# NGWPC/topoflow-glacier

Measured on AMD Instinct MI355X. Metric: cell-updates/sec (nx·ny·steps) on 8192² fp32 grid; % HBM roofline, higher is better.
Workload: dtype f32

## Files before the change

topoflow-glacier_amd/csrc/tfg_engine.hip:

```cpp
#include <hip/hip_runtime.h>
#include <mutex>

#include <algorithm>
#include <cmath>
#include <cstdio>
#include <cstdlib>
#include <atomic>
#include <chrono>
#include <cstring>
#include <new>
#include <string>
#include <type_traits>
#include <vector>

#include "../../include/tfg.h"
#include "tfg_physics.hpp"
#include "tfg_conduction.hpp"
#include "tfg_fused.hpp"
#include "tfg_hostbuf.hpp"

namespace {

using namespace tfg_kern;

// ... 978 lines not shown
  a.n_pad = h->n_pad;
  a.n_step = h->n_pad;
  return a;
}

template <class R, bool EXACT>
int launch_fused(tfg_handle* h, const tfg_uniforms* d_u, const StepAddr* d_t, int K, int blocks, size_t lds,
                 const IoArgs& io, bool ns, const Part* part = nullptr) {
  const hipStream_t stream = part ? part->stream : h->stream;
  KArgs a = step_args(h, K, io);
  if (part) {
    a.n = part->n_valid;
    a.n_step = part->cells;
  }
  const int64_t c0 = part ? part->c0 : 0;
  a.part_c0 = c0;
  const size_t rb = (size_t)c0 * h->rsz;
  const FusedBufs fb = {d_u, d_t, h->forc.bytes() + rb, h->stat.bytes() + rb, h->geo + c0,
                        h->catch_id ? h->catch_id + c0 : nullptr, h->st + c0, h->tot + c0, h->ring + c0,
                        h->hist.bytes() + rb, h->slab + (part ? part->slab_row0 : 0) * h->n_catch * 6,
                        h->qc ? h->qc.bytes() + rb : nullptr};
  const bool rd = !h->depths_derived;
  const bool ct = h->catch_id != nullptr;
  if constexpr (EXACT) {
    HIPCHK(h, launch_fused_exact(a, fb, rd, ct, h->qc_on, blocks, lds, stream));
    return TFG_OK;
  } else {
    const bool sat = h->dp.satterlund != 0;
    hipError_t e;
    if (h->flux_f64) e = sat ? launch_fused_fast<true, true>(a, fb, rd, ct, h->qc_on, ns, blocks, lds, stream)
                             : launch_fused_fast<true, false>(a, fb, rd, ct, h->qc_on, ns, blocks, lds, stream);
    else e = sat ? launch_fused_fast<false, true>(a, fb, rd, ct, h->qc_on, ns, blocks, lds, stream)
                 : launch_fused_fast<false, false>(a, fb, rd, ct, h->qc_on, ns, blocks, lds, stream);
    HIPCHK(h, e);
    return TFG_OK;
  }
}

}

template hipError_t tfg_kern::launch_fused_fast<false, false>(const KArgs&, const FusedBufs&, bool, bool, bool, bool, int,
                                                              size_t, hipStream_t);

extern "C" {

int tfg_abi_version(void) { return TFG_ABI_VERSION; }

#ifndef TFG_SRC_HASH
#define TFG_SRC_HASH "unknown"
#endif
#define TFG_STR2(x) #x
#define TFG_STR(x) TFG_STR2(x)
#if !defined(__HIP_DEVICE_COMPILE__)
__attribute__((used)) static const char tfg_build_tag[] =
    "libtfg abi=" TFG_STR(TFG_ABI_VERSION) " arch=gfx950 (hipcc) tfg-src-sha256=" TFG_SRC_HASH
    "; kernels: k_fused<float|double,exact|fast,...>, k_cell, k_cell_run, k_cell_many, k_diag_reduce, k_catch_series, k_band_series, k_forcing_expand, k_forcing_regrid, k_fill_synthetic";

const char* tfg_build_info(void) { return tfg_build_tag; }
#else
const char* tfg_build_info(void);
#endif

int tfg_device_count(int* count) {
  if (!count) return fail(nullptr, TFG_ERR_ARG, "null count");
  HIPCHK(nullptr, hipGetDeviceCount(count));
  return TFG_OK;
}

constexpr int64_t kPlaneSkew = 512;

int tfg_create(const tfg_params* p, int64_t ny, int64_t nx, int engine, int device, int n_frames,
               int hist_depth, int n_catch, tfg_handle** out) {
  if (!p || !out) return fail(nullptr, TFG_ERR_ARG, "null params/out");
  *out = nullptr;
  if (ny <= 0 || nx <= 0) return fail(nullptr, TFG_ERR_ARG, "grid must have ny, nx >= 1");
  if (ny > (1ll << 31) || nx > (1ll << 31))
    return fail(nullptr, TFG_ERR_ARG, "shard too large: ny and nx must stay below 2^31");
  if (engine != TFG_F32 && engine != TFG_F64) return fail(nullptr, TFG_ERR_ARG, "engine must be TFG_F32 or TFG_F64");
  if (n_frames < 1 || hist_depth < 1 || n_catch < 1) return fail(nullptr, TFG_ERR_ARG, "n_frames, hist_depth, n_catch must be >= 1");
  if (n_catch > 512) return fail(nullptr, TFG_ERR_ARG, "n_catch > 512 not supported");
  if (p->ring_len < 1) return fail(nullptr, TFG_ERR_ARG, "ring_len must be >= 1");
  if (!(p->dt > 0)) return fail(nullptr, TFG_ERR_ARG, "dt must be > 0");
  if (!(p->z0_air > 0.0 && p->z0_air < INFINITY)) return fail(nullptr, TFG_ERR_ARG, "z0_air must be finite and > 0");
  tfg_handle* h = new (std::nothrow) tfg_handle();
  if (!h) return fail(nullptr, TFG_ERR_ARG, "out of host memory");
  auto bail = [&](int rc) {
    g_err = h->err;
    tfg_destroy(h);
    return rc;
  };
  h->device = device;
  h->engine = engine;
  h->rsz = dtype_size(engine);
  h->ny = ny;
  h->nx = nx;
  h->n = ny * nx;
  h->n_pad = round_up(h->n, 64);
  h->n_pad += h->n_pad >= ((int64_t)1 << 20) ? kPlaneSkew : 0;
  if (h->n_pad * 8 >= (int64_t)1 << 32) {
    h->err = "shard too large: ny*nx must stay below 2^29 cells per device (32-bit field offsets)";
    g_err = h->err;
    delete h;
    return TFG_ERR_ARG;
  }
  h->n_frames = n_frames;
  h->hist_depth = hist_depth;
  h->n_catch = n_catch;
  h->ring_len = p->ring_len;
  derive_params(*p, h->dp);
  {
    const double rg = p->rho_ice * p->g;
    h->flow_gamma = 2.0 * p->glens_A / 5.0 * (rg * rg * rg);
    h->inv_cs = 1.0 / (p->rho_snow * p->Cp_snow);
    h->inv_ci = 1.0 / ((p->rho_ice * p->Cp_ice) * p->h_active_layer);
    h->h_active = p->h_active_layer;
  }
  if (hipSetDevice(device) != hipSuccess) { h->err = "hipSetDevice failed"; return bail(TFG_ERR_HIP); }
  hipDeviceProp_t prop;
  if (hipGetDeviceProperties(&prop, device) != hipSuccess) { h->err = "hipGetDeviceProperties failed"; return bail(TFG_ERR_HIP); }
  h->max_blocks = std::max(256, prop.multiProcessorCount * 512);
  h->max_blocks = (int)std::max<int64_t>(256, std::min<int64_t>(h->max_blocks, (256ll << 20) / ((int64_t)n_catch * 6 * 8)));
  while (h->max_blocks & (h->max_blocks - 1)) h->max_blocks &= h->max_blocks - 1;
  h->max_blocks = (int)std::min<int64_t>(h->max_blocks, (h->n_pad / kCellsPerThread + kBlock - 1) / kBlock);
  if (h->own_stream.create() != hipSuccess) { h->err = "stream create failed"; return bail(TFG_ERR_HIP); }
  h->stream = h->own_stream;
  const int64_t np = h->n_pad;
  const size_t rs = h->rsz;
  struct A { Buf<DevMem>* b; size_t bytes; } allocs[] = {
      {&h->forc, (size_t)n_frames * kNumForc * np * rs},
      {&h->stat, 3 * (size_t)np * rs},
      {&h->lwsw, 2 * (size_t)np * rs},
      {&h->geo, engine == TFG_F32 ? (size_t)np * (tfg::kGeoF * 4 + 2 * 8) : (size_t)np * tfg::kStaticPlanes * 8},
      {&h->st, (size_t)kNumState * np * 8},
      {&h->tot, (size_t)np * 8},
      {&h->ring, (size_t)p->ring_len * np * 4},
      {&h->hist, (size_t)hist_depth * kNumHist * np * rs},
      {&h->diag, (size_t)n_catch * 6 * 8},
      {&h->slab, (size_t)h->max_blocks * n_catch * 6 * 8},
      {&h->d_flag, (size_t)n_frames * kNumForc * 4},
  };
  for (auto& a : allocs) {
    const hipError_t e = (hipError_t)a.b->reserve(a.bytes);
    if (e != hipSuccess) {
      h->err = std::string("hipMalloc(") + std::to_string(a.bytes) + " B) failed: " + hipGetErrorString(e);
      return bail(TFG_ERR_HIP);
    }
    if (hipMemsetAsync(a.b->ptr, 0, a.bytes, h->stream) != hipSuccess) { h->err = "hipMemset failed"; return bail(TFG_ERR_HIP); }
  }
  if (hipStreamSynchronize(h->stream) != hipSuccess) { h->err = "sync failed"; return bail(TFG_ERR_HIP); }
  h->plane_state.assign((size_t)n_frames * kNumForc, kOk);
  *out = h;
  return TFG_OK;
}

int tfg_destroy(tfg_handle* h) {
  if (!h) return TFG_OK;
  (void)hipSetDevice(h->device);
  if (h->stream && h->stream != h->own_stream) (void)hipStreamSynchronize(h->stream);
  if (h->own_stream) (void)hipStreamSynchronize(h->own_stream);
  if (h->side) (void)hipStreamSynchronize(h->side);
  delete h;
  return TFG_OK;
}

int tfg_set_stream(tfg_handle* h, void* stream) {
  if (int rc_ = api_sync(h)) return rc_;
// ... 1563 lines not shown
```

topoflow-glacier_amd/csrc/tfg_fused.hpp:

```cpp
#pragma once

#include <hip/hip_runtime.h>

#include <algorithm>
#include <cmath>
#include <cstddef>
#include <cstdint>

#include "../../include/tfg.h"
#include "tfg_physics.hpp"

namespace tfg_kern {

using tfg::CellDiag;
using tfg::CellOut;
using tfg::CellState;
using tfg::CellStatic;
using tfg::CellStaticF;
using tfg::DevParams;

constexpr int kBlock = 256;
constexpr int kCellsPerThread = 1;
constexpr int kPrefetchFast = 2;
constexpr int kWaves = kBlock / 64;
// ... 89 lines not shown
#pragma unroll
    for (int off = 32; off >= 1; off >>= 1) {
      v0 += __shfl_xor(v0, off);
      v1 += __shfl_xor(v1, off);
      v2 += __shfl_xor(v2, off);
      v3 += __shfl_xor(v3, off);
      v4 += __shfl_xor(v4, off);
      m = tfg::npmax(m, __shfl_xor(m, off));
    }
    if (lane == leader) {
      double* b = wbins + 6 * c;
      b[0] += v0; b[1] += v1; b[2] += v2; b[3] += v3; b[4] += v4;
      b[5] = tfg::npmax(b[5], m);
    }
    pending &= ~__ballot(mine);
  }
}

#ifdef TFG_WG_TIMING
static __device__ unsigned long long g_wg_times[TFG_WG_TIMING][3];
#endif
constexpr int kMinWaves = 4;
constexpr int kMinWavesExact = 2;
constexpr int kMinWavesPrec = 4;
template <class R, bool EXACT, bool READ_DEPTHS, bool CATCH, bool QC, int C, bool NS = false, bool PREC = false,
          bool SAT = false>
__global__ __launch_bounds__(kBlock, EXACT ? kMinWavesExact : (PREC ? kMinWavesPrec : kMinWaves)) void k_fused(const KArgs a, const tfg_uniforms* __restrict__ uni,
                                                  const StepAddr* __restrict__ tab,
                                                  const R* __restrict__ forc,
                                                  const R* __restrict__ stat,
                                                  const float* __restrict__ geo,
                                                  const int32_t* __restrict__ catch_id,
                                                  double* __restrict__ st,
                                                  int64_t* __restrict__ tot,
                                                  int32_t* __restrict__ ring,
                                                  R* __restrict__ hist,
                                                  double* __restrict__ slab,
                                                  const R* __restrict__ qcf) {
  extern __shared__ double lds_bins[];
#ifdef TFG_WG_TIMING
  const unsigned long long t_wg0 = wall_clock64();
#endif
  const DevParams& p = a.p;
  const int nb = a.n_catch * 6;
  for (int i = threadIdx.x; i < kWaves * nb; i += kBlock) lds_bins[i] = ((i % 6) == 5) ? -INFINITY : 0.0;
  __syncthreads();
  double* wbins = lds_bins + (threadIdx.x >> 6) * nb;

  const int64_t n_pad = a.n_pad;
  const int64_t ngroups = a.n_step / C;
  const int64_t nchunks = (ngroups + kBlock - 1) / kBlock;
  const int64_t wg = blockIdx.x;
  const int64_t g0 = (wg * nchunks / gridDim.x) * kBlock;
  const int64_t g1 = std::min<int64_t>(((wg + 1) * nchunks / gridDim.x) * kBlock, ngroups);
  const int64_t trips = (g1 - g0 + kBlock - 1) / kBlock;
  const double* geo_d = reinterpret_cast<const double*>(geo + tfg::kGeoF * n_pad) + a.part_c0 / 2;
  float* const alb_f = reinterpret_cast<float*>(st + S_ALB * n_pad) - a.part_c0;

  CellDiag acc;
  diag_zero(acc);
  constexpr bool kAccLds = !EXACT && !CATCH;
  __shared__ double acc_lds[kAccLds ? 6 * kBlock : 1];
  auto acc_get = [&]() {
    const double* s = acc_lds + threadIdx.x;
    return CellDiag{s[0], s[kBlock], s[2 * kBlock], s[3 * kBlock], s[4 * kBlock], s[5 * kBlock]};
  };
  auto acc_put = [&](const CellDiag& d) {
    double* s = acc_lds + threadIdx.x;
    s[0] = d.P; s[kBlock] = d.PR; s[2 * kBlock] = d.PS; s[3 * kBlock] = d.SM; s[4 * kBlock] = d.IM; s[5 * kBlock] = d.Pmax;
  };
  if constexpr (kAccLds) acc_put(acc);

  for (int64_t it = 0; it < trips; ++it) {
    const int64_t g = g0 + it * kBlock + threadIdx.x;
    const bool in = g < g1;
    int32_t cid[C];
    CellDiag cacc[CATCH ? C : 1];
    if constexpr (CATCH) {
#pragma unroll
      for (int j = 0; j < C; ++j) { diag_zero(cacc[j]); cid[j] = 0; }
    }
    if (in) {
      const int64_t c0 = g * C;
      const uint32_t lc = (uint32_t)c0;
      CellStatic SX[EXACT ? C : 1];
      tfg::CellStaticF SF[EXACT ? 1 : C];
      if constexpr (EXACT) {
        const double* gx = reinterpret_cast<const double*>(geo);
        double v[tfg::kStaticPlanes][C];
#pragma unroll
        for (int f = 0; f < tfg::kStaticPlanes; ++f) dload<C>(gx + f * n_pad, lc, v[f]);
#pragma unroll
        for (int j = 0; j < C; ++j) SX[j] = {v[0][j], v[1][j], v[2][j], v[3][j], v[4][j], v[5][j], v[6][j]};
      } else {
        float gv[tfg::kGeoF][C];
#pragma unroll
        for (int f = 0; f < tfg::kGeoF; ++f) vload<float, C>(geo + f * n_pad, lc, gv[f]);
#pragma unroll
        for (int j = 0; j < C; ++j) SF[j] = {gv[0][j], gv[1][j], gv[2][j], gv[3][j], gv[4][j]};
      }
      CellState cs[C];
      {
        double v[C];
        dload<C>(st + S_HSWE * n_pad, lc, v);
#pragma unroll
        for (int j = 0; j < C; ++j) cs[j].h_swe = v[j];
        dload<C>(st + S_HIWE * n_pad, lc, v);
#pragma unroll
        for (int j = 0; j < C; ++j) cs[j].h_iwe = v[j];
        dload<C>(st + S_ECCS * n_pad, lc, v);
#pragma unroll
        for (int j = 0; j < C; ++j) cs[j].Eccs = v[j];
        dload<C>(st + S_ECCI * n_pad, lc, v);
#pragma unroll
        for (int j = 0; j < C; ++j) cs[j].Ecci = v[j];
        dload<C>(st + S_N * n_pad, lc, v);
#pragma unroll
        for (int j = 0; j < C; ++j) cs[j].n = v[j];
        if constexpr (EXACT) {
          dload<C>(st + S_ALB * n_pad, lc, v);
#pragma unroll
          for (int j = 0; j < C; ++j) cs[j].albedo = v[j];
        }
        if constexpr (READ_DEPTHS) {
          dload<C>(st + S_HSNOW * n_pad, lc, v);
#pragma unroll
          for (int j = 0; j < C; ++j) cs[j].h_snow = v[j];
          dload<C>(st + S_HICE * n_pad, lc, v);
#pragma unroll
          for (int j = 0; j < C; ++j) cs[j].h_ice = v[j];
        } else {
#pragma unroll
          for (int j = 0; j < C; ++j) {
            cs[j].h_snow = cs[j].h_swe * p.ws;
            cs[j].h_ice = cs[j].h_iwe * p.wi;
          }
        }
        int64_t t[C];
        lload<C>(tot, lc, t);
#pragma unroll
        for (int j = 0; j < C; ++j) cs[j].tot_q = t[j];
        if constexpr (!EXACT) {
          bool carried = false;
#pragma unroll
          for (int j = 0; j < C; ++j) {
            cs[j].albedo = 0.0;
            carried |= !(cs[j].h_snow > 0.0 || (cs[j].h_snow == 0.0 && (cs[j].h_ice > 0.0 || cs[j].h_ice == 0.0)));
          }
          if (__any(carried)) {
            float fa[C];
            vload<float, C>(alb_f, lc, fa);
#pragma unroll
            for (int j = 0; j < C; ++j) cs[j].albedo = (double)fa[j];
          }
        }
      }
      R qc[C];
      if constexpr (QC) vload<R, C>(qcf, lc, qc);
      else {
#pragma unroll
        for (int j = 0; j < C; ++j) qc[j] = (R)0;
      }
      tfg::DiagF df[EXACT ? 1 : C];
      if constexpr (!EXACT) {
#pragma unroll
        for (int j = 0; j < C; ++j) df[j] = {0.0f, 0.0f, 0.0f, 0.0f, 0.0f, 0.0f};
      }

      struct Frame { R P[C], T[C], Q[C], PA[C], UZ[C]; int32_t q[C]; };
      const char* const fbase = a.io_in ? static_cast<const char*>(a.io_in) : reinterpret_cast<const char*>(forc);
      auto fetch = [&](int k, Frame& f) {
        const StepAddr* ta = tab + (k < a.K ? k : a.K - 1);
        const int64_t fo = ta->forc, ro = ta->ring;
        const R* __restrict__ fr = reinterpret_cast<const R*>(fbase + fo);
        const int32_t* rs = reinterpret_cast<const int32_t*>(reinterpret_cast<const char*>(ring) + ro);
        static_assert(C == 1, "streamed step accesses are per cell");
        static_assert(sizeof(R) == 4 || sizeof(R) == 8, "R is float or double");
        const uint32_t oR = lane_off(lc * (uint32_t)sizeof(R));
        f.P[0] = sload(fr + F_P * n_pad, oR);
        f.T[0] = sload(fr + F_T * n_pad, oR);
        f.Q[0] = sload(fr + F_Q * n_pad, oR);
        f.PA[0] = sload(fr + F_PA * n_pad, oR);
        f.UZ[0] = sload(fr + F_UZ * n_pad, oR);
        f.q[0] = sload(rs, sizeof(R) == 4 ? oR : lane_off(lc * 4u));
      };
      auto advance = [&](int k, const Frame& f) {
        TFG_STEP_PARAMS(p);
        const tfg_uniforms* up = uni + k;
        const tfg_uniforms u = *up;
        int32_t qn[C];
        R o_hs[C], o_sm[C], o_hi[C], o_im[C], o_mt[C], o_rh[C];
#pragma unroll
        for (int j = 0; j < C; ++j) {
          if constexpr (EXACT) {
            CellOut o;
            CellDiag& d = CATCH ? cacc[j] : acc;
            const bool valid = (c0 + j) < a.n;
            const tfg::ParamsAsIs params{p};
            tfg::cell_step_exact<QC>(p, SX[j], u, (double)f.P[j], (double)f.T[j], (double)f.Q[j], (double)f.PA[j],
                                     (double)f.UZ[j], f.q[j], qn[j], cs[j], o, d, valid, (double)qc[j], params);
            o_hs[j] = (R)o.h_snow; o_sm[j] = (R)o.SM; o_hi[j] = (R)o.h_ice;
            o_im[j] = (R)o.IM; o_mt[j] = (R)o.M_total; o_rh[j] = (R)o.RH;
          } else {
            tfg::CellOutF o;
            tfg::cell_step_fast<QC, NS, PREC, SAT>(p, SF[j], up, u, geo_d, n_pad, c0 + j, (float)f.P[j], (float)f.T[j],
                                                   (float)f.Q[j], (float)f.PA[j], (float)f.UZ[j], f.q[j], qn[j], cs[j],
                                                   o, df[j], (float)qc[j]);
            o_hs[j] = (R)o.h_snow; o_sm[j] = (R)o.SM; o_hi[j] = (R)o.h_ice;
            o_im[j] = (R)o.IM; o_mt[j] = (R)o.M_total; o_rh[j] = (R)o.RH;
            asm volatile("" : "+v"(df[j].P), "+v"(df[j].PR), "+v"(df[j].PS), "+v"(df[j].Pmax));
          }
        }
        const uint32_t oR = lane_off(lc * (uint32_t)sizeof(R));
        const int64_t ro = tab[k].ring, ho = tab[k].hist;
        sstore(reinterpret_cast<int32_t*>(reinterpret_cast<char*>(ring) + ro), sizeof(R) == 4 ? oR : lane_off(lc * 4u), qn[0]);
        R* __restrict__ h = reinterpret_cast<R*>(reinterpret_cast<char*>(hist) + ho);
        sstore(h + H_HSNOW * n_pad, oR, o_hs[0]);
        sstore(h + H_SM * n_pad, oR, o_sm[0]);
        sstore(h + H_HICE * n_pad, oR, o_hi[0]);
        sstore(h + H_IM * n_pad, oR, o_im[0]);
        sstore(h + H_MTOT * n_pad, oR, o_mt[0]);
        sstore(h + H_RH * n_pad, oR, o_rh[0]);
      };
      constexpr int kAhead = (QC || NS || PREC) ? 1 : kPrefetchFast;
      Frame fa, fb;
      fetch(0, fa);
      if constexpr (EXACT) {
        for (int k = 0; k < a.K; ++k) {
          fetch(k + 1, fb);
          advance(k, fa);
          fa = fb;
        }
      } else if constexpr (kAhead == 2) {
        Frame fc;
        fetch(1, fb);
        int k = 0;
        if (a.K >= 3) {
          fetch(2, fc);
          advance(0, fa);
          fetch(3, fa);
          advance(1, fb);
          fetch(4, fb);
          advance(2, fc);
          for (k = 3; k + 3 <= a.K; k += 3) {
            fetch(k + 2, fc);
            advance(k, fa);
            fetch(k + 3, fa);
            advance(k + 1, fb);
            fetch(k + 4, fb);
            advance(k + 2, fc);
          }
        }
        if (k < a.K) {
          advance(k, fa);
          if (k + 1 < a.K) advance(k + 1, fb);
        }
      } else if constexpr (PREC && CATCH) {
        for (int k = 0; k < a.K; k += 2) {
          fetch(k + 1, fb);
          advance(k, fa);
          fetch(k + 2, fa);
          if (k + 1 < a.K) advance(k + 1, fb);
        }
      } else {
        int k = 0;
        if (a.K >= 2) {
          fetch(1, fb);
          advance(0, fa);
          fetch(2, fa);
          advance(1, fb);
          for (k = 2; k + 2 <= a.K; k += 2) {
            fetch(k + 1, fb);
            advance(k, fa);
            fetch(k + 2, fa);
            advance(k + 1, fb);
          }
        }
        if (k < a.K) advance(k, fa);
      }
      if (a.io_in) {
        const int fidx = uni[0].frame, hidx = uni[0].hist;
        R* __restrict__ fr = const_cast<R*>(forc) + (int64_t)fidx * kNumForc * n_pad;
        const uint32_t oR = lane_off(lc * (uint32_t)sizeof(R));
        sstore(fr + F_P * n_pad, oR, fa.P[0]);
        sstore(fr + F_T * n_pad, oR, fa.T[0]);
        sstore(fr + F_Q * n_pad, oR, fa.Q[0]);
        sstore(fr + F_PA * n_pad, oR, fa.PA[0]);
        sstore(fr + F_UZ * n_pad, oR, fa.UZ[0]);
        if (c0 < a.n) {
          const R* hs = hist + (int64_t)hidx * kNumHist * n_pad + c0;
          double* o = a.io_out + c0;
          const int64_t n = a.n;
          o[0 * n] = (double)hs[H_HSNOW * n_pad];
          o[1 * n] = cs[0].h_swe;
          o[2 * n] = (double)hs[H_SM * n_pad];
          o[3 * n] = (double)hs[H_HICE * n_pad];
          o[4 * n] = cs[0].h_iwe;
          o[5 * n] = (double)hs[H_IM * n_pad];
          o[6 * n] = (double)hs[H_MTOT * n_pad];
          o[7 * n] = (double)hs[H_RH * n_pad];
        }
      }
      if constexpr (CATCH) iload<C>(catch_id, lc, cid);
      if constexpr (!EXACT) {
        const double fP = p.da_m2 * p.dt, fSM = p.inv_dt_rhoLf * p.da_m2 * p.dt * 3600.0,
                     fIM = p.da_m2 * p.dt * 3600.0;
#pragma unroll
        for (int j = 0; j < C; ++j) {
          if ((c0 + j) < a.n) {
            CellDiag lsum;
            if constexpr (kAccLds) lsum = acc_get();
            CellDiag& d = CATCH ? cacc[j] : (kAccLds ? lsum : acc);
            d.P += (double)df[j].P * fP;
            d.PR += (double)df[j].PR * fP;
            d.PS += (double)df[j].PS * fP;
            d.SM += (double)df[j].Erem_s * fSM;
            d.IM += (double)df[j].IM * fIM;
            d.Pmax = tfg::npmax(d.Pmax, (double)df[j].Pmax);
            if constexpr (kAccLds) acc_put(lsum);
          }
        }
      }
      {
        double v[C];
#pragma unroll
        for (int j = 0; j < C; ++j) v[j] = cs[j].h_swe;
        dstore<C>(st + S_HSWE * n_pad, lc, v);
#pragma unroll
        for (int j = 0; j < C; ++j) v[j] = cs[j].h_iwe;
        dstore<C>(st + S_HIWE * n_pad, lc, v);
#pragma unroll
        for (int j = 0; j < C; ++j) v[j] = cs[j].Eccs;
        dstore<C>(st + S_ECCS * n_pad, lc, v);
#pragma unroll
        for (int j = 0; j < C; ++j) v[j] = cs[j].Ecci;
        dstore<C>(st + S_ECCI * n_pad, lc, v);
#pragma unroll
        for (int j = 0; j < C; ++j) v[j] = cs[j].n;
        dstore<C>(st + S_N * n_pad, lc, v);
        if constexpr (EXACT) {
#pragma unroll
          for (int j = 0; j < C; ++j) v[j] = cs[j].albedo;
          dstore<C>(st + S_ALB * n_pad, lc, v);
        } else {
          float fa[C];
#pragma unroll
          for (int j = 0; j < C; ++j) fa[j] = (float)cs[j].albedo;
          vstore<float, C>(alb_f, lc, fa);
        }
        int64_t t[C];
#pragma unroll
        for (int j = 0; j < C; ++j) t[j] = cs[j].tot_q;
        lstore<C>(tot, lc, t);
      }
    }
    if constexpr (CATCH) {
#pragma unroll
      for (int j = 0; j < C; ++j) {
        if constexpr (EXACT) diag_scale(cacc[j], p);
        wave_flush(wbins, cid[j], cacc[j], in);
      }
    }
// ... 87 lines not shown
```

topoflow-glacier_amd/csrc/tfg_physics.hpp:

```cpp
#pragma once
#include <hip/hip_runtime.h>
#include <stdint.h>

#include <type_traits>

#include "tfg_fastmath.hpp"

namespace tfg {

using tfg_fm::div_k;
using tfg_fm::div_r;
using tfg_fm::fdiv;
using tfg_fm::exp_k;
using tfg_fm::log_k;
using tfg_fm::atan_q;

constexpr double kOmega = (360.0 / 24.0) * (3.141592653589793 / 180.0);
constexpr double kInvOmega = 1.0 / kOmega;

struct DevParams {
  double dt, da_m2, T_rs, dust, F, one_minus_F_172, cloud_term;
  double rho_snow_Cp_snow;
  double rho_air_Cp_air;
  double rho_air_Lv;
// ... 639 lines not shown
  const double t = (sb * sa) / (cb * p.cos_lat - sb * p.sin_lat * ca);
  const double rt = 1.0 / sqrt(1.0 + t * t);
  const double dlon = atan(t);
  CellGeo g;
  g.f[0] = (float)(-p.negM_g / p.R * elev * 1.4426950408889634);
  g.f[1] = (float)sl;
  g.f[2] = (float)(cl * rt);
  g.f[3] = (float)(cl * t * rt);
  g.f[4] = (float)dlon;
  g.tan_eq = sl / cl;
  g.t_noon = -1.0 * dlon / p.omega;
  return g;
}

__device__ __noinline__ bool dark_exact(const DevParams& p, const double* __restrict__ geo_d, int64_t n_pad,
                                        int64_t i, const tfg_uniforms* __restrict__ up) {
#pragma clang fp contract(off)
  const double tan_eq = geo_d[i], t_noon = geo_d[n_pad + i];
  double arg = -1.0 * tan_eq * up->tan_d;
  arg = npmin(npmax(-1.0, arg), 1.0);
  const double ac = acos(arg);
  const double T_sr = npmax(-1.0 * ac / p.omega + t_noon, up->flat_sr);
  const double T_ss = npmin(ac / p.omega + t_noon, up->flat_ss);
  return (up->th <= T_sr) || (up->th >= T_ss);
}

__device__ __forceinline__ float fast_atanf(float x) {
  const float ax = fabsf(x);
  const bool big = ax > 1.0f;
  const float z = big ? frcp(ax) : ax;
  const float t = z * z;
  float u = 0.00282363896258175373f;
  u = fmaf(u, t, -0.0159569028764963150f);
  u = fmaf(u, t, 0.0425049886107444763f);
  u = fmaf(u, t, -0.0748900920152664185f);
  u = fmaf(u, t, 0.106347933411598206f);
  u = fmaf(u, t, -0.142027363181114197f);
  u = fmaf(u, t, 0.199926957488059998f);
  u = fmaf(u, t, -0.333331018686294556f);
  float r = fmaf(z * t, u, z);
  r = big ? 1.57079632679489662f - r : r;
  return copysignf(r, x);
}

__device__ __forceinline__ double sub_rounded(double h, double a, double b) {
#pragma clang fp contract(off)
  return h - a * b;
}
__device__ __forceinline__ double add_rounded(double h, double a, double b) {
#pragma clang fp contract(off)
  return h + a * b;
}

__device__ __forceinline__ float wet_bulb_f(float rh, float T_air) {
  const float a = T_air + rh, b = rh - 1.676331f;
  const float den = fmaf(a, b, 1.0f);
  float d = fast_atanf((T_air + 1.676331f) * frcp(den));
  if (den < 0.0f) d += copysignf(3.14159265358979f, a);
  const float x = 0.023101f * rh, x2 = x * x;
  float at = x * fmaf(fmaf(0.2f, x2, -0.333333333f), x2, 1.0f);
  const float t = fmaf(0.4f, rh, -1.0f);
  float a0 = fmaf(fmaf(fmaf(fmaf(fmaf(fmaf(-1.7216859760083025e-06f, t, 9.90594708127901e-06f), t,
                                       -5.9253852668916807e-05f), t, 0.0004237863759044558f), t,
                             -0.003739525331184268f), t, 0.046224694699048996f), t, 0.4634580910205841f);
  if (__any((rh < 0.0f) || (rh > 5.0f))) {
    const bool off = (rh < 0.0f) || (rh > 5.0f);
    a0 = off ? fast_atanf(0.151977f * __builtin_amdgcn_sqrtf(rh + 8.313659f)) : a0;
    at = off ? fast_atanf(x) : at;
  }
  return T_air * a0 + d + (0.00391838f * (rh * __builtin_amdgcn_sqrtf(rh))) * at - 4.86035f;
}

__device__ __forceinline__ float snowfall_cold(const DevParams& p, float P_snow, float rh, float T_air) {
  return p.f_c_eccs * P_snow * (p.f_T0 - wet_bulb_f(rh, T_air));
}

struct DiagF {
  float P, PR, PS, Erem_s, IM, Pmax;
};
struct CellOutF {
  float h_snow, SM, h_ice, IM, M_total, RH;
};

template <bool NS> __device__ __forceinline__ float nmax(float a, float b) { if constexpr (NS) return npmax(a, b); else return fmaxf(a, b); }
template <bool NS> __device__ __forceinline__ float nmin(float a, float b) { if constexpr (NS) return npmin(a, b); else return fminf(a, b); }
template <bool NS> __device__ __forceinline__ double dmax(double a, double b) { if constexpr (NS) return npmax(a, b); else return fmax(a, b); }
template <bool NS> __device__ __forceinline__ double dmin(double a, double b) { if constexpr (NS) return npmin(a, b); else return fmin(a, b); }

struct MeltF {
  double h_swe, h_iwe, Eccs, Ecci;
  float SM, IM, Erem_s, IM_int;
};
template <bool NS, class QT>
__device__ __forceinline__ MeltF melt_core(const DevParams& p, QT Q_sum, float P_snow, float RH, float T_air,
                                           double h_swe0, double h_iwe0, double Eccs0, double Ecci0,
                                           double h_ice_prev) {
  MeltF m;
  const double previous_swe = h_swe0;
  const double E_in = sizeof(QT) == 8 ? (double)Q_sum * p.dt : (double)(Q_sum * p.f_dt);
  const double E_rem_s = dmax<NS>(E_in - Eccs0, 0.0);
  m.Erem_s = (float)E_rem_s;
  double h_swe = add_rounded(h_swe0, (double)P_snow, p.dt);
  const double ts = dmin<NS>(E_rem_s * p.c_sm3600, h_swe);
  const double SM = ts * (1.0 / 3600.0);
  h_swe = dmax<NS>(sub_rounded(h_swe, SM, p.dt3600), 0.0);
  double Eccs = Eccs0;
  if (P_snow > 0.0f) Eccs = dmax<NS>(Eccs + (double)snowfall_cold(p, P_snow, RH, T_air) - E_in, 0.0);
  const double E_rem_i = dmax<NS>(E_in - Ecci0, 0.0);
  double IM = (h_swe == 0.0 && previous_swe == 0.0) ? E_rem_i * p.inv_dt_rhoLf : 0.0;
  double Ecci = dmax<NS>(Ecci0 - E_in, 0.0);
  Ecci = (h_ice_prev == 0.0) ? 0.0 : Ecci;
  IM = dmin<NS>(IM, h_iwe0 * p.inv_dt);
  m.IM_int = (float)IM;
  const double ti = dmin<NS>(IM * 3600.0, h_iwe0);
  IM = ti * (1.0 / 3600.0);
  const double h_iwe = dmax<NS>(sub_rounded(h_iwe0, IM, p.dt3600), 0.0);
  if (NS ? (P_snow <= 0.0f) : !(P_snow > 0.0f)) Eccs = dmax<NS>(Eccs - E_in, 0.0);
  Eccs = (h_swe * p.ws == 0.0) ? 0.0 : Eccs;
  m.h_swe = h_swe;
  m.h_iwe = h_iwe;
  m.Eccs = Eccs;
  m.Ecci = Ecci;
  m.SM = (float)SM;
  m.IM = (float)IM;
  return m;
}
template <bool NS, class QT>
__device__ __forceinline__ void melt_fast(const DevParams& p, QT Q_sum, float P_snow, float P_rain, float RH,
                                          float T_air, CellState& st, CellOutF& o, DiagF& d) {
  const MeltF m = melt_core<NS, QT>(p, Q_sum, P_snow, RH, T_air, st.h_swe, st.h_iwe, st.Eccs, st.Ecci, st.h_ice);
  d.Erem_s += m.Erem_s;
  d.IM += m.IM_int;
  const double h_snow = m.h_swe * p.ws;
  const double h_ice = m.h_iwe * p.wi;
  st.h_swe = m.h_swe;
  st.h_iwe = m.h_iwe;
  st.Eccs = m.Eccs;
  st.Ecci = m.Ecci;
  st.h_snow = h_snow;
  st.h_ice = h_ice;
  o.h_snow = (float)h_snow;
  o.h_ice = (float)h_ice;
  o.SM = m.SM;
  o.IM = m.IM;
  o.M_total = m.IM + m.SM + P_rain * (1.0f / 3600.0f);
  o.RH = RH;
}

template <bool QC, bool NANSAFE, bool PREC = false, bool SAT = false>
__device__ inline void cell_step_fast(const DevParams& p, const CellStaticF& g, const tfg_uniforms* __restrict__ up,
                                      const tfg_uniforms& u, const double* __restrict__ geo_d, int64_t n_pad,
                                      int64_t cell, float P, float T_air, float Hum_sp, float P_air, float uz,
                                      int32_t q_old, int32_t& q_new, CellState& st, CellOutF& o, DiagF& d, float qc) {
  constexpr bool NS = NANSAFE;
  const bool snow_pos = st.h_snow > 0.0, ice_pos = st.h_ice > 0.0;
  const float T_K = T_air + 273.15f;
  const float rT = frcp(T_K);
  const bool is_rain = T_air > p.f_T_rs_dn;
  const float P_rain = is_rain ? P : P * 0.0f;
  const float P_snow = (NS ? (T_air <= p.f_T_rs_dn) : !is_rain) ? P : P * 0.0f;
  d.P += P;
  d.Pmax = npmax(d.Pmax, P);
  d.PR += P_rain;
  d.PS += P_snow;
  const float rA = SAT ? rT : frcp(T_air + 237.3f);
  float inv_esat;
  if (!SAT) {
    inv_esat = (1.0f / 6.11f) * fexp2((-17.3f * kLog2e) * T_air * rA);
  } else {
    inv_esat = 100.0f * fexp2((2353.0f * rT - 11.4f) * 3.3219280948873626f);
  }
  double Td = T_air, e64 = 0.0, Tsd = 0.0, dTd = 0.0;
  float e_air, T_dew, T_surf, dTs;
  if constexpr (PREC) {
    e64 = ((double)Hum_sp * (double)P_air) * rcp_nr1(fma((double)Hum_sp, p.d_ome100, p.d_eps100));
    const double Ld = tfg_fm::log_p(e64 * (1.0 / 6.1121));
    const double Tdew = (257.14 * Ld) * rcp_nr1(18.678 - Ld);
    Tsd = (snow_pos || ice_pos) ? dmin<NS>(Tdew, 0.0) : Tdew;
    dTd = Td - Tsd;
    e_air = (float)e64;
    T_dew = (float)Tdew;
    T_surf = (float)Tsd;
    dTs = (float)dTd;
  } else {
    e_air = Hum_sp * P_air * frcp_nr(p.f_eps100 + p.f_ome100 * Hum_sp);
    const float log_term = flog2_nr(e_air * (1.0f / 6.1121f)) * kLn2;
    T_dew = 257.14f * log_term * frcp_nr(18.678f - log_term);
    T_surf = (snow_pos || ice_pos) ? nmin<NS>(T_dew, 0.0f) : T_dew;
    dTs = T_air - T_surf;
  }
  const float RH = e_air * inv_esat;
  const float ly2 = flog2(nmax<NS>((p.f_z - (float)st.h_snow) * p.f_inv_z0s, p.f_l2min));
  std::conditional_t<PREC, double, float> Qh, Qe;
  if constexpr (PREC) {
    const double uzd = uz;
    double botd = (uzd * uzd) * (Td + 273.15);
    if (botd == 0.0) botd = 0.01;
    const double top = p.gz * dTd;
    const double L2 = fma((double)ly2, (double)ly2 + 2.0 * p.d_l2k, p.d_l2kk);
    const bool stable = top > 0.0;
    const double num = stable ? botd : fma(-10.0, top, botd);
    const double den = stable ? fma(10.0, top, botd) : botd;
    const double Dhd = (uzd * p.d_k2) * num * rcp_nr1(L2 * den);
    Qh = (p.rho_air_Cp_air * Dhd) * dTd;
    const double x_es = (-p.d_es_k * dTd) * rcp_nr1((Tsd + p.d_es_c) * (Td + p.d_es_c));
    const double ded = e64 * (1.0 - tfg_fm::exp_p(x_es));
    const double s0 = fma((double)g.ek * 0.69314718055994531, rcp_nr1(Td + 273.15), -tfg_fm::kP0Center);
    const bool far = !(fabs(s0) <= tfg_fm::kP0Half);
    double p0f;
    if (__builtin_expect(__any(far), 0)) {
      TFG_FM_RARE();
      p0f = tfg_fm::exp_p(s0);
      if (__any(!far)) {
        TFG_FM_RARE();
        p0f = far ? p0f : tfg_fm::exp_near(s0);
      }
    } else {
      p0f = tfg_fm::exp_near(s0);
    }
    Qe = (p.d_qe * Dhd) * ded * p0f;
  } else {
    float bot = (uz * uz) * T_K;
    if (bot == 0.0f) bot = 0.01f;
    const float Ri = p.f_gz * dTs * frcp(bot);
    const float L2sq = fmaf(ly2, ly2 + p.f_l2k2, p.f_l2kk);
    const float Dn = uz * p.f_k2 * frcp(L2sq);
    const float Dh = (Ri > 0.0f) ? Dn * frcp(fmaf(10.0f, Ri, 1.0f)) : Dn * fmaf(-10.0f, Ri, 1.0f);
    const float rS = frcp(T_surf + (SAT ? 273.15f : 237.3f));
    const float xs2 = (SAT ? -7816.4968f : -5922.6815f) * dTs * rS * rA;
    const float de = fmaf(-e_air, fexp2(xs2), e_air);
    Qh = p.f_rho_air_Cp_air * Dh * dTs;
    Qe = p.f_qe * Dh * de * fexp2(g.ek * rT);
  }
  {
    const float sq = P_snow * p.f_qfac;
    const int32_t q = (int32_t)__float2int_rn(fminf(fmaxf(sq, -2147483520.0f), 2147483520.0f));
    q_new = NS ? ((sq == sq) ? q : kWindowNan) : q;
  }
  if constexpr (NS) {
    st.tot_q += window_tot(q_new) - window_tot(q_old);
    st.n = window_days(st.n, st.tot_q, p.thr_q, p.days_per_dt);
  } else {
    st.tot_q += (int64_t)q_new - (int64_t)q_old;
    st.n = (st.tot_q >= p.thr_q) ? 0.0 : st.n + p.days_per_dt;
  }
  float albedo;
  {
    const float r = (T_air > 0.0f) ? (0.12f * kLog2e) : (0.05f * kLog2e);
    const float snow_albedo = 0.4f + 0.44f * fexp2(-(float)st.n * r);
    float a = snow_pos ? snow_albedo : (float)st.albedo;
    if (st.h_snow == 0.0 && ice_pos) a = 0.3f;
    if (st.h_snow == 0.0 && st.h_ice == 0.0) a = 0.15f;
    st.albedo = (double)a;
    albedo = a;
  }
  float K_cs = 0.0f;
  if (!u.flat_dark) {
    const float w = fexp2((0.0614f * kLog2e) * T_dew);
    const float tau = nmin<NS>(nmax<NS>(fexp2(fmaf(u.tau_c1, w, u.tau_c0)) - p.f_dust, 0.0f), 1.0f);
    const float gam_s = p.f_1pdust - fexp2(fmaf(u.gam_c1, w, u.gam_c0));
    const float cwl = u.cos_wth_f * g.cc - u.sin_wth_f * g.cs;
    const float K_ET = fmaxf(fmaf(u.kc_f, cwl, u.ks_f * g.sl), 0.0f);
    const float kf = u.k_et_flat_f;
    const float K_dif = 0.5f * gam_s * kf;
    const float K_bs = 0.5f * gam_s * albedo * fmaf(tau, kf, K_dif);
    K_cs = tau * K_ET + K_dif + K_bs;
    {
      const float dv = fmaf(g.sl, u.tan_d_f, cwl);
      const float ax = fabsf(u.omega_th_f + g.dlon);
      const float mpi = ax - 3.14159265358979f;
      bool dark;
      if (!(fabsf(dv) >= 1e-5f) || !(fabsf(mpi) >= 1e-4f)) {
        dark = dark_exact(p, geo_d, n_pad, cell, up);
      } else {
        dark = (mpi > 0.0f) || (dv <= 0.0f);
      }
      if (dark) K_cs = 0.0f;
    }
  }
  const float Qn_SW = K_cs * (1.0f - albedo);
  float em_m1;
  if (!SAT) {
    if constexpr (PREC) {
      em_m1 = 0.0f;
    } else {
      const float em_r = fexp2(flog2(e_air * p.f_em_sc * rT) * (1.0f / 7.0f));
      em_m1 = fmaf(p.f_ccFs, em_r, p.f_Fm1);
    }
  } else {
    em_m1 = 1.08f * (1.0f - fexp2(-kLog2e * fexp2(flog2(e_air) * (T_K * (1.0f / 2016.0f))))) - 1.0f;
  }
  std::conditional_t<PREC, double, float> Qn_LW;
  if constexpr (PREC) {
    const double TaK = Td + 273.15, TsK = Tsd + 273.15;
    const double emd_m1 = SAT ? (double)em_m1
                                       : fma(p.one_minus_F_172 * p.cloud_term, root7_p((e64 * 0.1) * rcp_nr1(TaK)), p.F - 1.0);
    const double ta2d = TaK * TaK;
    Qn_LW = p.em_surf_sigma * fma(emd_m1, ta2d * ta2d, dTd * (TaK + TsK) * fma(TsK, TsK, ta2d));
  } else {
    const float T_surf_K = T_surf + 273.15f;
    const float ta2 = T_K * T_K;
    const float d4 = dTs * (T_K + T_surf_K) * fmaf(T_surf_K, T_surf_K, ta2);
    Qn_LW = p.f_em_surf_sigma * fmaf(em_m1, ta2 * ta2, d4);
  }
  std::conditional_t<PREC, double, float> Q_sum;
  if constexpr (PREC) Q_sum = (((double)Qn_SW + Qn_LW) + Qh) + Qe + (QC ? (double)qc : 0.0);
  else {
    Q_sum = fmaf(K_cs, 1.0f - albedo, Qn_LW) + Qh + Qe;
    if constexpr (QC) Q_sum = Q_sum + qc;
  }

  melt_fast<NS, decltype(Q_sum)>(p, Q_sum, P_snow, P_rain, RH, T_air, st, o, d);
#if defined(TFG_DEBUG_TERMS)
  o.h_snow = Qn_SW;
  o.SM = (float)Qn_LW;
  o.h_ice = (float)Qh;
  o.IM = (float)Qe;
  o.M_total = P_snow > 0.0f ? snowfall_cold(p, P_snow, RH, T_air) : 0.0f;
  o.RH = (float)Q_sum;
#endif
}

}
```

Baseline: 137.5 billion.

## Derive snow/ice depth state from water equivalents in lean fp32 path

In the lean fp32 path (not EXACT, not PREC, depths not read), the per-step h_snow and h_ice double state is no longer stored. Zero and positive tests use h_swe/h_iwe instead, and a float copy of h_snow is carried between steps. The change also adds inline-asm v_min/v_max helpers and keeps the step offset and precipitation value in a register through opaque asm, so fewer registers and instructions are spent per step. A host-side check now requires water/snow/ice density ratios >= 1 so that the derived zero tests stay equivalent. It also adds a TFG_MEM_ONLY debug stub.

```diff
diff --git a/topoflow-glacier_amd/csrc/tfg_engine.hip b/topoflow-glacier_amd/csrc/tfg_engine.hip
--- a/topoflow-glacier_amd/csrc/tfg_engine.hip
+++ b/topoflow-glacier_amd/csrc/tfg_engine.hip
@@ -1084,6 +1084,11 @@
   if (p->ring_len < 1) return fail(nullptr, TFG_ERR_ARG, "ring_len must be >= 1");
   if (!(p->dt > 0)) return fail(nullptr, TFG_ERR_ARG, "dt must be > 0");
   if (!(p->z0_air > 0.0 && p->z0_air < INFINITY)) return fail(nullptr, TFG_ERR_ARG, "z0_air must be finite and > 0");
+  if (engine == TFG_F32) {
+    const double ws = p->rho_H2O / p->rho_snow, wi = p->rho_H2O / p->rho_ice;
+    if (!(ws >= 1.0 && ws < INFINITY && wi >= 1.0 && wi < INFINITY))
+      return fail(nullptr, TFG_ERR_ARG, "the fp32 engine needs 0 < rho_snow <= rho_H2O and 0 < rho_ice <= rho_H2O");
+  }
   tfg_handle* h = new (std::nothrow) tfg_handle();
   if (!h) return fail(nullptr, TFG_ERR_ARG, "out of host memory");
   auto bail = [&](int rc) {
diff --git a/topoflow-glacier_amd/csrc/tfg_fused.hpp b/topoflow-glacier_amd/csrc/tfg_fused.hpp
--- a/topoflow-glacier_amd/csrc/tfg_fused.hpp
+++ b/topoflow-glacier_amd/csrc/tfg_fused.hpp
@@ -195,7 +195,7 @@
     }
     if (in) {
       const int64_t c0 = g * C;
-      const uint32_t lc = (uint32_t)c0;
+      uint32_t lc = (uint32_t)c0;
       CellStatic SX[EXACT ? C : 1];
       tfg::CellStaticF SF[EXACT ? 1 : C];
       if constexpr (EXACT) {
@@ -282,6 +282,20 @@
 
       struct Frame { R P[C], T[C], Q[C], PA[C], UZ[C]; int32_t q[C]; };
       const char* const fbase = a.io_in ? static_cast<const char*>(a.io_in) : reinterpret_cast<const char*>(forc);
+      constexpr bool kLean = !EXACT && !PREC;
+      uint32_t step_oR = lc * (uint32_t)sizeof(R);
+      auto step_off = [&]() -> uint32_t {
+        if constexpr (!kLean) {
+          return lane_off(lc * (uint32_t)sizeof(R));
+        } else {
+          asm volatile("" : "+v"(step_oR));
+          return step_oR;
+        }
+      };
+      constexpr bool kDerived = kLean && !READ_DEPTHS;
+      float hs_f[C];
+#pragma unroll
+      for (int j = 0; j < C; ++j) hs_f[j] = (float)cs[j].h_snow;
       auto fetch = [&](int k, Frame& f) {
         const StepAddr* ta = tab + (k < a.K ? k : a.K - 1);
         const int64_t fo = ta->forc, ro = ta->ring;
@@ -289,7 +303,7 @@
         const int32_t* rs = reinterpret_cast<const int32_t*>(reinterpret_cast<const char*>(ring) + ro);
         static_assert(C == 1, "streamed step accesses are per cell");
         static_assert(sizeof(R) == 4 || sizeof(R) == 8, "R is float or double");
-        const uint32_t oR = lane_off(lc * (uint32_t)sizeof(R));
+        const uint32_t oR = step_off();
         f.P[0] = sload(fr + F_P * n_pad, oR);
         f.T[0] = sload(fr + F_T * n_pad, oR);
         f.Q[0] = sload(fr + F_Q * n_pad, oR);
@@ -316,15 +330,17 @@
             o_im[j] = (R)o.IM; o_mt[j] = (R)o.M_total; o_rh[j] = (R)o.RH;
           } else {
             tfg::CellOutF o;
-            tfg::cell_step_fast<QC, NS, PREC, SAT>(p, SF[j], up, u, geo_d, n_pad, c0 + j, (float)f.P[j], (float)f.T[j],
-                                                   (float)f.Q[j], (float)f.PA[j], (float)f.UZ[j], f.q[j], qn[j], cs[j],
-                                                   o, df[j], (float)qc[j]);
+            float P_in = (float)f.P[j];
+            if constexpr (kLean) asm volatile("" : "+v"(P_in));
+            tfg::cell_step_fast<QC, NS, PREC, SAT, kDerived>(p, SF[j], up, u, geo_d, n_pad, c0 + j, P_in,
+                                                             (float)f.T[j], (float)f.Q[j], (float)f.PA[j], (float)f.UZ[j],
+                                                             f.q[j], qn[j], cs[j], o, df[j], (float)qc[j], hs_f[j]);
             o_hs[j] = (R)o.h_snow; o_sm[j] = (R)o.SM; o_hi[j] = (R)o.h_ice;
             o_im[j] = (R)o.IM; o_mt[j] = (R)o.M_total; o_rh[j] = (R)o.RH;
             asm volatile("" : "+v"(df[j].P), "+v"(df[j].PR), "+v"(df[j].PS), "+v"(df[j].Pmax));
           }
         }
-        const uint32_t oR = lane_off(lc * (uint32_t)sizeof(R));
+        const uint32_t oR = step_off();
         const int64_t ro = tab[k].ring, ho = tab[k].hist;
         sstore(reinterpret_cast<int32_t*>(reinterpret_cast<char*>(ring) + ro), sizeof(R) == 4 ? oR : lane_off(lc * 4u), qn[0]);
         R* __restrict__ h = reinterpret_cast<R*>(reinterpret_cast<char*>(hist) + ho);
@@ -391,6 +407,7 @@
         }
         if (k < a.K) advance(k, fa);
       }
+      if constexpr (kLean) lc = step_oR / (uint32_t)sizeof(R);
       if (a.io_in) {
         const int fidx = uni[0].frame, hidx = uni[0].hist;
         R* __restrict__ fr = const_cast<R*>(forc) + (int64_t)fidx * kNumForc * n_pad;
diff --git a/topoflow-glacier_amd/csrc/tfg_physics.hpp b/topoflow-glacier_amd/csrc/tfg_physics.hpp
--- a/topoflow-glacier_amd/csrc/tfg_physics.hpp
+++ b/topoflow-glacier_amd/csrc/tfg_physics.hpp
@@ -745,6 +745,21 @@
   float h_snow, SM, h_ice, IM, M_total, RH;
 };
 
+__device__ __forceinline__ float hw_max_sv(float s, float v) {
+  float r;
+  asm("v_max_f32 %0, %1, %2" : "=v"(r) : "s"(s), "v"(v));
+  return r;
+}
+__device__ __forceinline__ float hw_min0(float v) {
+  float r;
+  asm("v_min_f32 %0, 0, %1" : "=v"(r) : "v"(v));
+  return r;
+}
+__device__ __forceinline__ double hw_min(double a, double b) {
+  double r;
+  asm("v_min_f64 %0, %1, %2" : "=v"(r) : "v"(a), "v"(b));
+  return r;
+}
 template <bool NS> __device__ __forceinline__ float nmax(float a, float b) { if constexpr (NS) return npmax(a, b); else return fmaxf(a, b); }
 template <bool NS> __device__ __forceinline__ float nmin(float a, float b) { if constexpr (NS) return npmin(a, b); else return fminf(a, b); }
 template <bool NS> __device__ __forceinline__ double dmax(double a, double b) { if constexpr (NS) return npmax(a, b); else return fmax(a, b); }
@@ -754,7 +769,7 @@
   double h_swe, h_iwe, Eccs, Ecci;
   float SM, IM, Erem_s, IM_int;
 };
-template <bool NS, class QT>
+template <bool NS, class QT, bool DER = false>
 __device__ __forceinline__ MeltF melt_core(const DevParams& p, QT Q_sum, float P_snow, float RH, float T_air,
                                            double h_swe0, double h_iwe0, double Eccs0, double Ecci0,
                                            double h_ice_prev) {
@@ -772,14 +787,16 @@
   const double E_rem_i = dmax<NS>(E_in - Ecci0, 0.0);
   double IM = (h_swe == 0.0 && previous_swe == 0.0) ? E_rem_i * p.inv_dt_rhoLf : 0.0;
   double Ecci = dmax<NS>(Ecci0 - E_in, 0.0);
-  Ecci = (h_ice_prev == 0.0) ? 0.0 : Ecci;
+  Ecci = (DER ? (h_iwe0 == 0.0) : (h_ice_prev == 0.0)) ? 0.0 : Ecci;
   IM = dmin<NS>(IM, h_iwe0 * p.inv_dt);
   m.IM_int = (float)IM;
-  const double ti = dmin<NS>(IM * 3600.0, h_iwe0);
+  double ti;
+  if constexpr (NS || sizeof(QT) == 8) ti = dmin<NS>(IM * 3600.0, h_iwe0);
+  else ti = hw_min(IM * 3600.0, h_iwe0);
   IM = ti * (1.0 / 3600.0);
   const double h_iwe = dmax<NS>(sub_rounded(h_iwe0, IM, p.dt3600), 0.0);
   if (NS ? (P_snow <= 0.0f) : !(P_snow > 0.0f)) Eccs = dmax<NS>(Eccs - E_in, 0.0);
-  Eccs = (h_swe * p.ws == 0.0) ? 0.0 : Eccs;
+  Eccs = (DER ? (h_swe == 0.0) : (h_swe * p.ws == 0.0)) ? 0.0 : Eccs;
   m.h_swe = h_swe;
   m.h_iwe = h_iwe;
   m.Eccs = Eccs;
@@ -788,10 +805,11 @@
   m.IM = (float)IM;
   return m;
 }
-template <bool NS, class QT>
+template <bool NS, class QT, bool DER = false>
 __device__ __forceinline__ void melt_fast(const DevParams& p, QT Q_sum, float P_snow, float P_rain, float RH,
-                                          float T_air, CellState& st, CellOutF& o, DiagF& d) {
-  const MeltF m = melt_core<NS, QT>(p, Q_sum, P_snow, RH, T_air, st.h_swe, st.h_iwe, st.Eccs, st.Ecci, st.h_ice);
+                                          float T_air, CellState& st, CellOutF& o, DiagF& d, float& h_snow_f) {
+  const MeltF m = melt_core<NS, QT, DER>(p, Q_sum, P_snow, RH, T_air, st.h_swe, st.h_iwe, st.Eccs, st.Ecci,
+                                         DER ? 0.0 : st.h_ice);
   d.Erem_s += m.Erem_s;
   d.IM += m.IM_int;
   const double h_snow = m.h_swe * p.ws;
@@ -800,23 +818,45 @@
   st.h_iwe = m.h_iwe;
   st.Eccs = m.Eccs;
   st.Ecci = m.Ecci;
-  st.h_snow = h_snow;
-  st.h_ice = h_ice;
+  if constexpr (!DER) {
+    st.h_snow = h_snow;
+    st.h_ice = h_ice;
+  }
   o.h_snow = (float)h_snow;
   o.h_ice = (float)h_ice;
+  h_snow_f = o.h_snow;
   o.SM = m.SM;
   o.IM = m.IM;
   o.M_total = m.IM + m.SM + P_rain * (1.0f / 3600.0f);
   o.RH = RH;
 }
 
-template <bool QC, bool NANSAFE, bool PREC = false, bool SAT = false>
+template <bool QC, bool NANSAFE, bool PREC = false, bool SAT = false, bool DER = false>
 __device__ inline void cell_step_fast(const DevParams& p, const CellStaticF& g, const tfg_uniforms* __restrict__ up,
                                       const tfg_uniforms& u, const double* __restrict__ geo_d, int64_t n_pad,
                                       int64_t cell, float P, float T_air, float Hum_sp, float P_air, float uz,
-                                      int32_t q_old, int32_t& q_new, CellState& st, CellOutF& o, DiagF& d, float qc) {
+                                      int32_t q_old, int32_t& q_new, CellState& st, CellOutF& o, DiagF& d, float qc,
+                                      float& h_snow_f) {
   constexpr bool NS = NANSAFE;
-  const bool snow_pos = st.h_snow > 0.0, ice_pos = st.h_ice > 0.0;
+#if defined(TFG_MEM_ONLY)
+  {
+    const float s = P + T_air + Hum_sp + P_air + uz + qc;
+    q_new = q_old + 1;
+    st.tot_q += 1;
+    d.P += s;
+    o.h_snow = s;
+    o.SM = s + 1.0f;
+    o.h_ice = s + 2.0f;
+    o.IM = s + 3.0f;
+    o.M_total = s + 4.0f;
+    o.RH = s + 5.0f;
+    h_snow_f = s;
+    return;
+  }
+#endif
+  const bool snow_pos = (DER ? st.h_swe : st.h_snow) > 0.0, ice_pos = (DER ? st.h_iwe : st.h_ice) > 0.0;
+  const bool snow_zero = (DER ? st.h_swe : st.h_snow) == 0.0, ice_zero = (DER ? st.h_iwe : st.h_ice) == 0.0;
+  const float h_snow_prev = DER ? h_snow_f : (float)st.h_snow;
   const float T_K = T_air + 273.15f;
   const float rT = frcp(T_K);
   const bool is_rain = T_air > p.f_T_rs_dn;
@@ -849,11 +889,17 @@
     e_air = Hum_sp * P_air * frcp_nr(p.f_eps100 + p.f_ome100 * Hum_sp);
     const float log_term = flog2_nr(e_air * (1.0f / 6.1121f)) * kLn2;
     T_dew = 257.14f * log_term * frcp_nr(18.678f - log_term);
-    T_surf = (snow_pos || ice_pos) ? nmin<NS>(T_dew, 0.0f) : T_dew;
+    float T_neg;
+    if constexpr (NS) T_neg = npmin(T_dew, 0.0f);
+    else T_neg = hw_min0(T_dew);
+    T_surf = (snow_pos || ice_pos) ? T_neg : T_dew;
     dTs = T_air - T_surf;
   }
   const float RH = e_air * inv_esat;
-  const float ly2 = flog2(nmax<NS>((p.f_z - (float)st.h_snow) * p.f_inv_z0s, p.f_l2min));
+  const float ly_arg = (p.f_z - h_snow_prev) * p.f_inv_z0s;
+  float ly2;
+  if constexpr (NS || PREC) ly2 = flog2(nmax<NS>(ly_arg, p.f_l2min));
+  else ly2 = flog2(hw_max_sv(p.f_l2min, ly_arg));
   std::conditional_t<PREC, double, float> Qh, Qe;
   if constexpr (PREC) {
     const double uzd = uz;
@@ -912,8 +958,8 @@
     const float r = (T_air > 0.0f) ? (0.12f * kLog2e) : (0.05f * kLog2e);
     const float snow_albedo = 0.4f + 0.44f * fexp2(-(float)st.n * r);
     float a = snow_pos ? snow_albedo : (float)st.albedo;
-    if (st.h_snow == 0.0 && ice_pos) a = 0.3f;
-    if (st.h_snow == 0.0 && st.h_ice == 0.0) a = 0.15f;
+    if (snow_zero && ice_pos) a = 0.3f;
+    if (snow_zero && ice_zero) a = 0.15f;
     st.albedo = (double)a;
     albedo = a;
   }
@@ -973,7 +1019,7 @@
     if constexpr (QC) Q_sum = Q_sum + qc;
   }
 
-  melt_fast<NS, decltype(Q_sum)>(p, Q_sum, P_snow, P_rain, RH, T_air, st, o, d);
+  melt_fast<NS, decltype(Q_sum), DER>(p, Q_sum, P_snow, P_rain, RH, T_air, st, o, d, h_snow_f);
 #if defined(TFG_DEBUG_TERMS)
   o.h_snow = Qn_SW;
   o.SM = (float)Qn_LW;
```

New measurement: 138.1 billion (median of 6 runs). Within noise of the previous version (+0.4%).
